# simone7monaco/NO-NODE-comparison

Measured on NVIDIA B200. Metric: train trajectories/s (EGNO 20-body, fwd+bwd+Adam), higher is better.
Workload: dtype f32

## Files before the change

### include/nbody_b200.h

```cpp
#ifndef NBODY_B200_H
#define NBODY_B200_H

#include <stdint.h>

#ifdef __cplusplus
extern "C" {
#endif

#define NB_HIDDEN 64
#define NB_MAX_EDGE_FEA 4
#define NB_MAX_T 16
#define NB_MAX_NODES 100

#define NB_OK 0
#define NB_ERR_INVALID (-1)
#define NB_ERR_CUDA (-2)

typedef struct NbEgnoConfig {
  int32_t B;
  int32_t N;
  int32_t T;
  int32_t n_layers;
  int32_t num_modes;
  int32_t in_node_nf;
// ... 64 lines not shown
                      const float* saved, const float* g_x_out, const float* g_h_out, const float* g_v_out,
                      float* grad_params, float* g_x_in, float* g_v_in, float* g_h_in, float* workspace, void* stream);

int64_t nb_segno_input_grad_workspace_floats(const NbSegnoConfig* cfg);
int nb_segno_backward_ex(const NbSegnoConfig* cfg, const float* params, const float* his, const float* edge_attr,
                         const float* saved, const float* g_x_out, const float* g_h_out, const float* g_v_out,
                         float* grad_params, float* g_x_in, float* g_v_in, float* g_h_in, float* g_his,
                         float* g_edge_attr, float* workspace, float* input_grad_workspace, void* stream);

int nb_segno_embed_forward(const NbSegnoConfig* cfg, const float* params, int64_t rows, const float* his, float* h,
                           void* stream);
int64_t nb_segno_embed_backward_workspace_floats(const NbSegnoConfig* cfg, int64_t rows);
int nb_segno_embed_backward(const NbSegnoConfig* cfg, int64_t rows, const float* his, const float* g_h, float* grad_params,
                            float* workspace, void* stream);
int nb_segno_merge_forward(int32_t mode, int64_t n, int32_t L, int32_t frame, const float* h_all, const float* x_all,
                           const float* v_all, const float* h_int, const float* x_int, const float* v_int,
                           const float* attn_params, float* h_out, float* x_out, float* v_out, float* alpha, void* stream);
int64_t nb_segno_merge_backward_workspace_floats(int64_t n);
int nb_segno_merge_backward(int32_t mode, int64_t n, int32_t L, int32_t frame, const float* h_all, const float* x_all,
                            const float* v_all, const float* h_int, const float* x_int, const float* v_int,
                            const float* attn_params, const float* alpha, const float* g_h, const float* g_x,
                            const float* g_v, float* g_h_all, float* g_x_all, float* g_v_all, float* g_h_int,
                            float* g_x_int, float* g_v_int, float* g_attn, int32_t accumulate, float* workspace,
                            void* stream);
int nb_accumulate(int64_t n, float* dst, const float* src, void* stream);

int nb_check_canonical_edges(const int64_t* row, const int64_t* col, int64_t n_edges, int32_t B, int32_t N,
                             int32_t* flag_dev, void* stream);


int nb_egcl_edge_forward(int32_t n_gt, int32_t B, int32_t N, int32_t n_edge_fea, int32_t clamp_per_edge,
                         const float* x, const float* P, const float* Q, const float* edge_fea, const float* w1,
                         int32_t ldw1, int32_t col_rad, int32_t col_ef, const float* W2, const float* b2,
                         const float* W3, const float* b3, const float* w4, const float* b4, float* M, float* Fsum,
                         void* stream);

int64_t nb_egcl_edge_backward_workspace_floats(int32_t n_gt, int32_t N);
int nb_egcl_edge_backward(int32_t n_gt, int32_t B, int32_t N, int32_t n_edge_fea, int32_t clamp_per_edge,
                          const float* x, const float* P, const float* Q, const float* edge_fea, const float* w1,
                          int32_t ldw1, int32_t col_rad, int32_t col_ef, const float* W2, const float* b2,
                          const float* W3, const float* b3, const float* w4, const float* b4, const float* gM,
                          const float* gFsum, float* gP, float* gQ, float* gx, float* gw, float* workspace,
                          void* stream);

long long nb_launch_count(void);
#define NB_PROFILE_CATEGORIES 8
int nb_profile_enable(int enable);
int nb_profile_read(double* ms , long long* counts );

int nb_set_edge_impl(int impl);
int nb_get_edge_impl(void);
int nb_set_edge_fwd3(int on);
int nb_get_edge_fwd3(void);
int nb_set_node_impl(int impl);
int nb_get_node_impl(void);
int nb_set_node_fused(int on);
int nb_get_node_fused(void);
int nb_set_segno_fused(int on);
int nb_get_segno_fused(void);

int nb_nbody_features(int32_t B, int32_t N, int32_t with_charge, const float* loc, const float* vel, const float* charges,
                      const float* edge_attr_o, float* nodes, float* loc_mean, float* edge_attr, void* stream);
int nb_nbody_energy(int32_t kind, int32_t F, int32_t B, int32_t N, float G, const float* loc, const float* vel,
                    const float* charges, float* energy, void* stream);

int64_t nb_traj_mse_workspace_floats(int32_t T);
int nb_traj_mse(int32_t T, int64_t rows, int32_t target_layout, int32_t only_first, const float* pred, const float* target,
                float* losses, float* loss, float* grad, float* workspace, void* stream);

int nb_sim_charged(int32_t B, int32_t N, int32_t T, int32_t sample_freq, double dt, double strength, double max_force,
                   double box_size, const double* loc0, const double* vel0, const double* charges, double* loc, double* vel,
                   void* stream);
int nb_sim_gravity(int32_t B, int32_t N, int32_t T, int32_t sample_freq, double dt, double G, double softening,
                   const double* pos0, const double* vel0, const double* mass, double* pos, double* vel, double* force,
                   void* stream);

int nb_adam_step(int64_t n, float* params, const float* grads, float* exp_avg, float* exp_avg_sq, float* step,
                 int32_t tick, double lr, double beta1, double beta2, double eps, double weight_decay, double grad_scale,
                 void* stream);
int nb_adam_step_peers(int64_t n, float* params, const void* const* peer_grads, int32_t npeer, float* exp_avg,
                       float* exp_avg_sq, float* step, int32_t tick, double lr, double beta1, double beta2, double eps,
                       double weight_decay, double grad_scale, void* stream);

int nb_tc_selftest(int32_t mode, const float* A, const float* W, float* out, void* stream);

int nb_silu_selftest(int64_t n, const float* x, float* out_mufu, float* out_fma, void* stream);

#ifdef __cplusplus
}
#endif
#endif
```

### no-node-comparison_b200/_cabi.py

```python
from __future__ import annotations

import ctypes as C

c_f = C.c_void_p


class NbEgnoConfig(C.Structure):
    _fields_ = [("B", C.c_int32), ("N", C.c_int32), ("T", C.c_int32), ("n_layers", C.c_int32),
                ("num_modes", C.c_int32), ("in_node_nf", C.c_int32), ("in_edge_nf", C.c_int32),
                ("time_emb_dim", C.c_int32), ("use_time_conv", C.c_int32), ("num_inputs", C.c_int32)]


class NbSegnoConfig(C.Structure):
    _fields_ = [("B", C.c_int32), ("N", C.c_int32), ("T", C.c_int32), ("in_node_nf", C.c_int32),
                ("in_edge_nf", C.c_int32), ("recurrent", C.c_int32), ("coords_weight", C.c_float),
                ("h_given", C.c_int32)]


EXPORTS = {
    "nb_version": (C.c_int, []),
    "nb_last_error": (C.c_char_p, []),
    "nb_egno_param_count": (C.c_int64, [C.POINTER(NbEgnoConfig)]),
    "nb_segno_param_count": (C.c_int64, [C.POINTER(NbSegnoConfig)]),
    "nb_egno_saved_floats": (C.c_int64, [C.POINTER(NbEgnoConfig)]),
    "nb_egno_workspace_floats": (C.c_int64, [C.POINTER(NbEgnoConfig), C.c_int]),
    "nb_segno_saved_floats": (C.c_int64, [C.POINTER(NbSegnoConfig)]),
    "nb_segno_workspace_floats": (C.c_int64, [C.POINTER(NbSegnoConfig), C.c_int]),
    "nb_egno_forward": (C.c_int, [C.POINTER(NbEgnoConfig)] + [c_f] * 14),
    "nb_egno_backward": (C.c_int, [C.POINTER(NbEgnoConfig)] + [c_f] * 15),
    "nb_segno_forward": (C.c_int, [C.POINTER(NbSegnoConfig)] + [c_f] * 11),
    "nb_segno_backward": (C.c_int, [C.POINTER(NbSegnoConfig)] + [c_f] * 13),
    "nb_egno_input_grad_workspace_floats": (C.c_int64, [C.POINTER(NbEgnoConfig)]),
    "nb_egno_backward_ex": (C.c_int, [C.POINTER(NbEgnoConfig)] + [c_f] * 19),
    "nb_egno_forward_ft": (C.c_int, [C.POINTER(NbEgnoConfig)] + [c_f] * 14),
    "nb_egno_backward_ft": (C.c_int, [C.POINTER(NbEgnoConfig)] + [c_f] * 21),
    "nb_segno_input_grad_workspace_floats": (C.c_int64, [C.POINTER(NbSegnoConfig)]),
    "nb_segno_backward_ex": (C.c_int, [C.POINTER(NbSegnoConfig)] + [c_f] * 16),
    "nb_segno_embed_forward": (C.c_int, [C.POINTER(NbSegnoConfig), c_f, C.c_int64, c_f, c_f, c_f]),
    "nb_segno_embed_backward_workspace_floats": (C.c_int64, [C.POINTER(NbSegnoConfig), C.c_int64]),
    "nb_segno_embed_backward": (C.c_int, [C.POINTER(NbSegnoConfig), C.c_int64] + [c_f] * 5),
    "nb_segno_merge_forward": (C.c_int, [C.c_int32, C.c_int64, C.c_int32, C.c_int32] + [c_f] * 12),
    "nb_segno_merge_backward_workspace_floats": (C.c_int64, [C.c_int64]),
    "nb_segno_merge_backward": (C.c_int, [C.c_int32, C.c_int64, C.c_int32, C.c_int32] + [c_f] * 18 + [C.c_int32, c_f, c_f]),
    "nb_accumulate": (C.c_int, [C.c_int64, c_f, c_f, c_f]),
    "nb_check_canonical_edges": (C.c_int, [c_f, c_f, C.c_int64, C.c_int32, C.c_int32, c_f, c_f]),
    "nb_egcl_edge_forward": (C.c_int, [C.c_int32] * 5 + [c_f] * 5 + [C.c_int32] * 3 + [c_f] * 9),
    "nb_egcl_edge_backward_workspace_floats": (C.c_int64, [C.c_int32, C.c_int32]),
    "nb_egcl_edge_backward": (C.c_int, [C.c_int32] * 5 + [c_f] * 5 + [C.c_int32] * 3 + [c_f] * 14),
    "nb_nbody_features": (C.c_int, [C.c_int32] * 3 + [c_f] * 8),
    "nb_nbody_energy": (C.c_int, [C.c_int32] * 4 + [C.c_float] + [c_f] * 5),
    "nb_sim_charged": (C.c_int, [C.c_int32] * 4 + [C.c_double] * 4 + [c_f] * 6),
    "nb_sim_gravity": (C.c_int, [C.c_int32] * 4 + [C.c_double] * 3 + [c_f] * 7),
    "nb_traj_mse_workspace_floats": (C.c_int64, [C.c_int32]),
    "nb_traj_mse": (C.c_int, [C.c_int32, C.c_int64, C.c_int32, C.c_int32] + [c_f] * 7),
    "nb_adam_step": (C.c_int, [C.c_int64] + [c_f] * 5 + [C.c_int32] + [C.c_double] * 6 + [c_f]),
    "nb_adam_step_peers": (C.c_int, [C.c_int64, c_f, C.POINTER(C.c_void_p), C.c_int32] + [c_f] * 3 + [C.c_int32] + [C.c_double] * 6 + [c_f]),
    "nb_launch_count": (C.c_longlong, []),
    "nb_profile_enable": (C.c_int, [C.c_int]),
    "nb_profile_read": (C.c_int, [C.POINTER(C.c_double), C.POINTER(C.c_longlong)]),
    "nb_set_edge_impl": (C.c_int, [C.c_int]),
    "nb_set_node_impl": (C.c_int, [C.c_int]),
    "nb_get_node_impl": (C.c_int, []),
    "nb_set_node_fused": (C.c_int, [C.c_int]),
    "nb_get_node_fused": (C.c_int, []),
    "nb_set_segno_fused": (C.c_int, [C.c_int]),
    "nb_get_segno_fused": (C.c_int, []),
    "nb_get_edge_impl": (C.c_int, []),
    "nb_set_edge_fwd3": (C.c_int, [C.c_int]),
    "nb_get_edge_fwd3": (C.c_int, []),
    "nb_tc_selftest": (C.c_int, [C.c_int32, c_f, c_f, c_f, c_f]),
    "nb_silu_selftest": (C.c_int, [C.c_int64, c_f, c_f, c_f, c_f]),
}


def declare(lib: C.CDLL) -> C.CDLL:
    for name, (res, args) in EXPORTS.items():
        fn = getattr(lib, name)
        fn.restype = res
        fn.argtypes = args
    return lib
```

### no-node-comparison_b200/csrc/nb_spectral.cuh

```cuda
#pragma once
#include "nb_common.cuh"

#define NB_MAX_MODES (NB_MAX_T / 2 + 1)
#define NB_MAX_COEF (2 * NB_MAX_MODES - 1)

struct NbTwiddle {
  int T, modes, ncoef;
  int nyq;
  float c[NB_MAX_MODES][NB_MAX_T];
  float s[NB_MAX_MODES][NB_MAX_T];
};

__host__ __device__ __forceinline__ int nb_coef_index(const NbTwiddle& tw, int m) { return m == 0 ? 0 : 2 * m - 1; }

struct NbDftArgs {
  NbTwiddle tw;
  int Nn0;
  const float* x;
  float* coef;
  const float* ycoef;
  float* out;
  const float* gout;
  float* gycoef;
  const float* gcoef;
// ... 323 lines not shown
      const int idx = tid + (half * 8 + it) * 256;
      w0[it] = __ldg(reinterpret_cast<const float2*>(W + (int64_t)idx * modes * 2));
      w1[it] = modes > 1 ? __ldg(reinterpret_cast<const float2*>(W + (int64_t)idx * modes * 2 + 2)) : make_float2(0.f, 0.f);
    }
#pragma unroll
    for (int it = 0; it < 8; ++it) {
      const int idx = tid + (half * 8 + it) * 256;
      const int i = idx >> 6, o = idx & 63;
      if (B0) {
        B0[idx] = w0[it].x;
        B1[idx] = w1[it].x;
        B2[idx] = w1[it].y;
      }
      if (T0) {
        T0[o * NB_TCV_LDT + i] = w0[it].x;
        T1[o * NB_TCV_LDT + i] = w1[it].x;
        T2[o * NB_TCV_LDT + i] = w1[it].y;
      }
    }
  }
}

__device__ __forceinline__ void nb_tconv_mix(const float* As, const float* B0, const float* B1, const float* B2, int ldb,
                                             int r, int c4, bool has1, bool pair1, float4& o0, float4& o1, float4& o2) {
  o0 = o1 = o2 = make_float4(0.f, 0.f, 0.f, 0.f);
  const float* a0 = As + r * NB_TCV_LDA;
  const float* a1 = a0 + NB_TCV_ROWS * NB_TCV_LDA;
  const float* a2 = a1 + NB_TCV_ROWS * NB_TCV_LDA;
#pragma unroll 2
  for (int k0 = 0; k0 < NB_H; k0 += 4) {
    const float4 v0 = nb_ld4(a0 + k0);
    const float4 v1 = has1 ? nb_ld4(a1 + k0) : make_float4(0.f, 0.f, 0.f, 0.f);
    const float4 v2 = pair1 ? nb_ld4(a2 + k0) : make_float4(0.f, 0.f, 0.f, 0.f);
    const float x0[4] = {v0.x, v0.y, v0.z, v0.w}, x1[4] = {v1.x, v1.y, v1.z, v1.w}, x2[4] = {v2.x, v2.y, v2.z, v2.w};
#pragma unroll
    for (int kk = 0; kk < 4; ++kk) {
      const int k = k0 + kk;
      o0 = nb_f4_fma(x0[kk], nb_ld4(B0 + k * ldb + c4 * 4), o0);
      if (has1) {
        const float4 b1 = nb_ld4(B1 + k * ldb + c4 * 4);
        o1 = nb_f4_fma(x1[kk], b1, o1);
        if (pair1) {
          const float4 b2 = nb_ld4(B2 + k * ldb + c4 * 4);
          o1 = nb_f4_fma(x2[kk], b2, o1);
          o2 = nb_f4_fma(x1[kk], b2, o2);
          o2 = nb_f4_fma(-x2[kk], b1, o2);
        }
      }
    }
  }
}

template <int MAXT>
__global__ void __launch_bounds__(256, 3) k_tconv_fwd(NbTconvArgs a) {
  NB_PDL_ENTER();
  NB_DYN_SMEM(sm);
  float* B0 = sm;
  float* B1 = B0 + NB_H * NB_H;
  float* B2 = B1 + NB_H * NB_H;
  float* As = B2 + NB_H * NB_H;
  const int tid = threadIdx.x, r = tid >> 4, c4 = tid & 15;
  const NbTwiddle& tw = a.tw;
  const bool has1 = tw.modes > 1, pair1 = has1 && tw.nyq != 1;
  const int64_t plane = (int64_t)a.Nn0 * NB_H;
  const float invT = 1.0f / (float)tw.T;
  const int ngroups = (a.Nn0 + NB_TCV_ROWS - 1) / NB_TCV_ROWS;
  float4 xs[MAXT];
  {
    const int row = blockIdx.x * NB_TCV_ROWS + r;
    const bool act = (int)blockIdx.x < ngroups && row < a.Nn0;
    const int64_t off = (int64_t)row * NB_H + c4 * 4;
#pragma unroll
    for (int t = 0; t < MAXT; ++t)
      if (t < tw.T) xs[t] = act ? nb_ld4(a.x + t * plane + off) : make_float4(0.f, 0.f, 0.f, 0.f);
  }
  nb_tconv_stage_w(B0, B1, B2, nullptr, nullptr, nullptr, a.W, tw.modes, tid);
  for (int grp = blockIdx.x; grp < ngroups; grp += gridDim.x) {
    const int row = grp * NB_TCV_ROWS + r;
    const bool act = row < a.Nn0;
    const int64_t off = (int64_t)row * NB_H + c4 * 4;
    if (grp != (int)blockIdx.x) {
#pragma unroll
      for (int t = 0; t < MAXT; ++t)
        if (t < tw.T) xs[t] = act ? nb_ld4(a.x + t * plane + off) : make_float4(0.f, 0.f, 0.f, 0.f);
    }
    float4 C0 = make_float4(0.f, 0.f, 0.f, 0.f), C1 = C0, S1 = C0;
#pragma unroll
    for (int t = 0; t < MAXT; ++t)
      if (t < tw.T) {
        C0 = nb_f4_fma(tw.c[0][t], xs[t], C0);
        if (has1) C1 = nb_f4_fma(tw.c[1][t], xs[t], C1);
        if (pair1) S1 = nb_f4_fma(tw.s[1][t], xs[t], S1);
      }
    __syncthreads();
    nb_st4(As + r * NB_TCV_LDA + c4 * 4, C0);
    nb_st4(As + (NB_TCV_ROWS + r) * NB_TCV_LDA + c4 * 4, C1);
    nb_st4(As + (2 * NB_TCV_ROWS + r) * NB_TCV_LDA + c4 * 4, S1);
    __syncthreads();
    float4 P0, P1, Q1;
    nb_tconv_mix(As, B0, B1, B2, NB_H, r, c4, has1, pair1, P0, P1, Q1);
    if (act) {
      const float s1 = pair1 ? 2.f * invT : invT;
      uint32_t m0 = 0u, m1 = 0u;
#pragma unroll
      for (int t = 0; t < MAXT; ++t)
        if (t < tw.T) {
          float4 y = make_float4(P0.x * invT, P0.y * invT, P0.z * invT, P0.w * invT);
          if (has1) y = nb_f4_fma(s1 * tw.c[1][t], P1, y);
          if (pair1) y = nb_f4_fma(-s1 * tw.s[1][t], Q1, y);
          nb_st4(a.out + t * plane + off, make_float4(xs[t].x + nb_leaky(y.x), xs[t].y + nb_leaky(y.y),
                                                      xs[t].z + nb_leaky(y.z), xs[t].w + nb_leaky(y.w)));
          const uint32_t bits = (y.x > 0.f ? 1u : 0u) | (y.y > 0.f ? 2u : 0u) | (y.z > 0.f ? 4u : 0u) | (y.w > 0.f ? 8u : 0u);
          if (t < 8) m0 |= bits << (4 * t);
          else m1 |= bits << (4 * (t - 8));
        }
      if (a.mask) {
        a.mask[((int64_t)row * 16 + c4) * 2] = m0;
        a.mask[((int64_t)row * 16 + c4) * 2 + 1] = m1;
      }
    }
  }
}

template <int MAXT>
__global__ void __launch_bounds__(256, 2) k_tconv_bwd(NbTconvArgs a) {
  NB_PDL_ENTER();
  NB_DYN_SMEM(sm);
  float* T0 = sm;
  float* T1 = T0 + NB_H * NB_TCV_LDT;
  float* T2 = T1 + NB_H * NB_TCV_LDT;
  float* As = T2 + NB_H * NB_TCV_LDT;
  const int tid = threadIdx.x, r = tid >> 4, c4 = tid & 15;
  const NbTwiddle& tw = a.tw;
  const bool has1 = tw.modes > 1, pair1 = has1 && tw.nyq != 1;
  const int64_t plane = (int64_t)a.Nn0 * NB_H;
  const float invT = 1.0f / (float)tw.T;
  const float s1 = pair1 ? 2.f * invT : invT;
  const int ngroups = (a.Nn0 + NB_TCV_ROWS - 1) / NB_TCV_ROWS;
  float4 gq[MAXT];
  {
    const int row = blockIdx.x * NB_TCV_ROWS + r;
    const bool act = (int)blockIdx.x < ngroups && row < a.Nn0;
    const int64_t off = (int64_t)row * NB_H + c4 * 4;
#pragma unroll
    for (int t = 0; t < MAXT; ++t)
      if (t < tw.T) gq[t] = act ? nb_ld4(a.gout + t * plane + off) : make_float4(0.f, 0.f, 0.f, 0.f);
  }
  nb_tconv_stage_w(nullptr, nullptr, nullptr, T0, T1, T2, a.W, tw.modes, tid);
  for (int grp = blockIdx.x; grp < ngroups; grp += gridDim.x) {
    const int row = grp * NB_TCV_ROWS + r;
    const bool act = row < a.Nn0;
    const int64_t off = (int64_t)row * NB_H + c4 * 4;
    if (grp != (int)blockIdx.x) {
#pragma unroll
      for (int t = 0; t < MAXT; ++t)
        if (t < tw.T) gq[t] = act ? nb_ld4(a.gout + t * plane + off) : make_float4(0.f, 0.f, 0.f, 0.f);
    }
    const uint32_t mk0 = act ? a.mask[((int64_t)row * 16 + c4) * 2] : 0u, mk1 = act ? a.mask[((int64_t)row * 16 + c4) * 2 + 1] : 0u;
    float4 C0 = make_float4(0.f, 0.f, 0.f, 0.f), C1 = C0, S1 = C0, gP0 = C0, gP1 = C0, gQ1 = C0;
#pragma unroll
    for (int t = 0; t < MAXT; ++t)
      if (t < tw.T) {
        const float4 xv = act ? nb_ld4(a.x + t * plane + off) : make_float4(0.f, 0.f, 0.f, 0.f);
        C0 = nb_f4_fma(tw.c[0][t], xv, C0);
        if (has1) C1 = nb_f4_fma(tw.c[1][t], xv, C1);
        if (pair1) S1 = nb_f4_fma(tw.s[1][t], xv, S1);
        const uint32_t bits = (t < 8 ? mk0 >> (4 * t) : mk1 >> (4 * (t - 8))) & 15u;
        const float4 g = gq[t];
        const float4 gy = make_float4(g.x * ((bits & 1u) ? 1.f : 0.01f), g.y * ((bits & 2u) ? 1.f : 0.01f),
                                      g.z * ((bits & 4u) ? 1.f : 0.01f), g.w * ((bits & 8u) ? 1.f : 0.01f));
        gP0 = nb_f4_fma(invT * tw.c[0][t], gy, gP0);
        if (has1) gP1 = nb_f4_fma(s1 * tw.c[1][t], gy, gP1);
        if (pair1) gQ1 = nb_f4_fma(-s1 * tw.s[1][t], gy, gQ1);
      }
    if (act) {
      nb_st4(a.coef + off, C0);
      if (has1) nb_st4(a.coef + plane + off, C1);
      if (pair1) nb_st4(a.coef + 2 * plane + off, S1);
      nb_st4(a.gycoef + off, gP0);
      if (has1) nb_st4(a.gycoef + plane + off, gP1);
      if (pair1) nb_st4(a.gycoef + 2 * plane + off, gQ1);
    }
    __syncthreads();
    nb_st4(As + r * NB_TCV_LDA + c4 * 4, gP0);
    nb_st4(As + (NB_TCV_ROWS + r) * NB_TCV_LDA + c4 * 4, gP1);
    nb_st4(As + (2 * NB_TCV_ROWS + r) * NB_TCV_LDA + c4 * 4, gQ1);
    __syncthreads();
    float4 gC0, gC1, gS1;
    nb_tconv_mix(As, T0, T1, T2, NB_TCV_LDT, r, c4, has1, pair1, gC0, gC1, gS1);
    if (act) {
#pragma unroll
      for (int t = 0; t < MAXT; ++t)
        if (t < tw.T) {
          float4 g = gq[t];
          g = nb_f4_fma(tw.c[0][t], gC0, g);
          if (has1) g = nb_f4_fma(tw.c[1][t], gC1, g);
          if (pair1) g = nb_f4_fma(tw.s[1][t], gS1, g);
          nb_st4(a.gx + t * plane + off, g);
        }
    }
  }
}
```

### no-node-comparison_b200/csrc/nbody_b200.cu

```cuda
#include <math.h>
#include <stdarg.h>
#include <stdio.h>
#include <string.h>

#include "nb_common.cuh"
#include "nb_node.cuh"
#include "nb_spectral.cuh"
#include "nb_rollout.cuh"
#include "nb_sim.cuh"
#include "nb_edge.cuh"
#include "nb_tc.cuh"
#include "nb_edge_tc.cuh"
#include "nb_edge_sel.cuh"
#include "nb_node_tc.cuh"
#include "nb_segno_fused.cuh"
#include "nb_merge.cuh"
#include "nb_egno_node.cuh"
#include <cstdlib>

#define NB_LAUNCH_COUNTED(...)                             \
  do {                                                     \
    __atomic_fetch_add(&g_launches, 1LL, __ATOMIC_RELAXED); \
    NB_LAUNCH(__VA_ARGS__);                                \
  } while (0)
// ... 948 lines not shown
}

static int egno_tc_mix(const EgnoCtx& X, int l, const float* coef, float* ycoef) {
  const int modes = X.c->num_modes;
  const float* W = X.params + X.lo.L[l].tc;
  const int64_t plane = X.Nn0 * NB_H;
  const int64_t sk = (int64_t)NB_H * modes * 2, sn = (int64_t)modes * 2;
  NbGemmArgs jobs[2 * NB_MAX_T];
  int nj = 0;
  for (int m = 0; m < modes; ++m) {
    int ci = nb_coef_index(X.tw, m);
    const float* Wr = W + m * 2;
    const float* Wi = W + m * 2 + 1;
    if (m == 0 || m == X.tw.nyq) {
      NbGemmArgs a = gemm_args((int)X.Nn0);
      a.nsrc = 1; a.src[0] = gsrc(coef + ci * plane, NB_H, 0, Wr, sk, sn);
      a.out = ycoef + ci * plane;
      jobs[nj++] = a;
    } else {
      NbGemmArgs a = gemm_args((int)X.Nn0);
      a.nsrc = 2;
      a.src[0] = gsrc(coef + ci * plane, NB_H, 0, Wr, sk, sn);
      a.src[1] = gsrc(coef + (ci + 1) * plane, NB_H, 0, Wi, sk, sn);
      a.out = ycoef + ci * plane;
      jobs[nj++] = a;
      NbGemmArgs b = gemm_args((int)X.Nn0);
      b.nsrc = 2;
      b.src[0] = gsrc(coef + ci * plane, NB_H, 0, Wi, sk, sn);
      b.src[1] = gsrc(coef + (ci + 1) * plane, NB_H, 0, Wr, sk, sn, -1.f);
      b.out = ycoef + (ci + 1) * plane;
      jobs[nj++] = b;
    }
  }
  return launch_gemm_batch(jobs, nj, X.st, true);
}

static NbDftArgs dft_args(const EgnoCtx& X) {
  NbDftArgs d;
  memset(&d, 0, sizeof(d));
  d.tw = X.tw;
  d.Nn0 = (int)X.Nn0;
  return d;
}

static inline bool egno_tconv_fused(const EgnoCtx& X) { return X.c->num_modes <= 2; }
static NbTconvArgs tconv_args(const EgnoCtx& X, int l) {
  NbTconvArgs t;
  memset(&t, 0, sizeof(t));
  t.tw = X.tw;
  t.Nn0 = (int)X.Nn0;
  t.W = X.params + X.lo.L[l].tc;
  return t;
}
static inline int tconv_grid(const EgnoCtx& X, int per_sm) {
  return imin(cdiv(X.Nn0, NB_TCV_ROWS), (int64_t)per_sm * nb_num_sms());
}

static bool egno_node_fused(const EgnoCtx& X) {
#ifndef NB_EMU
  static int off = -1;
  if (off < 0) { const char* e = getenv("NB_B200_EGNO_NODE_FUSED"); off = (e && e[0] == '0') ? 1 : 0; }
  return !off && g_node_fused && g_node_impl == 1 && g_wimg.n == EGNO_WIMG_PER_LAYER * X.c->n_layers;
#else
  (void)X;
  return false;
#endif
}

static int egno_pq(const EgnoCtx& X, int l, const float* h1, float* P, float* Q) {
  const EgnoLayerOff& L = X.lo.L[l];
  const int E = X.lo.E;
#ifndef NB_EMU
  if (egno_node_fused(X)) {
    NbEgnoPairArgs pa;
    memset(&pa, 0, sizeof(pa));
    pa.rows = (int)X.Nn; pa.img = g_wimg.img[EGNO_WIMG_PER_LAYER * l]; pa.A0 = h1; pa.bias = X.params + L.e_b1; pa.O0 = P; pa.O1 = Q;
    NB_SET_SMEM(k_egno_pair<true>, NB_EPR_SMEM);
    int pi = prof_begin(2, X.st);
    NB_LAUNCH_COUNTED(k_egno_pair<true>, (unsigned)imin(cdiv(X.Nn, NB_TILE), 2 * nb_num_sms()), NB_THREADS, NB_EPR_SMEM, X.st, pa);
    prof_end(2, pi, X.st);
    return nb_check_launch("k_egno_pair");
  }
#endif
  NbGemmArgs a = gemm_args((int)X.Nn);
  a.nsrc = 1; a.src[0] = gsrc(h1, NB_H, 0, X.params + L.e_w1 + 1, 1, E);
  a.bias = X.params + L.e_b1; a.out = P;
  NbGemmArgs b = gemm_args((int)X.Nn);
  b.nsrc = 1; b.src[0] = gsrc(h1, NB_H, 0, X.params + L.e_w1 + 1 + NB_H, 1, E);
  b.out = Q;
  NbGemmArgs ab[2] = {a, b};
  return launch_gemm_batch(ab, 2, X.st);
}

static NbEdgeW egno_edge_w(const EgnoCtx& X, int l) {
  const EgnoLayerOff& L = X.lo.L[l];
  NbEdgeW w;
  w.W1 = X.params + L.e_w1; w.ldw1 = X.lo.E; w.col_rad = 0; w.col_ef = 1 + 2 * NB_H;
  w.W2 = X.params + L.e_w2; w.b2 = X.params + L.e_b2; w.W3 = X.params + L.c_w1; w.b3 = X.params + L.c_b1;
  w.w4 = X.params + L.c_w2; w.b4 = X.params + L.c_b2;
  return w;
}

static int egno_forward(const NbEgnoConfig* cfg, const float* params, const float* x, const float* nodes,
                        const float* edge_fea, const float* v, const float* loc_mean, const EgnoTimes& times,
                        float* x_out, float* v_out, float* h_out, float* saved, float* workspace, void* stream) {
  NB_RANGE("nb_egno_forward");
  EgnoCtx X;
  NB_TRY(egno_ctx_init(&X, cfg, params, stream));
// ... 2 lines not shown
  const int64_t nh = align64(Nn * NB_H), cf = egno_coef_floats(cfg), lf = align64(egno_layer_floats(Nn, X.Nn0));
  WimgGuard wimg_guard;
  NB_TRY(egno_weight_images(X, workspace));
  float* ttab = workspace + wimg_floats(EGNO_WIMG_PER_LAYER * Ln);
  float* P = ttab + egno_table_floats(cfg);
  float* Q = P + nh;
  float* coef = Q + nh;
  float* ycoef = coef + cf;
  float* infer = ycoef + cf;
  auto bufs = [&](int l) { return egno_layer_bufs(saved ? saved + (int64_t)l * lf : infer + (int64_t)(l & 1) * lf, Nn); };

  EgnoLayerBufs b0 = bufs(0);
  {
    NbEmbedArgs e;
    NB_TRY(egno_embed_inputs(cfg, X.lo, e, nodes, times, ttab, P, Q, stream));
    {
      NbGemmArgs ga = gemm_args((int)Nn);
      ga.nsrc = 1; ga.src[0] = gsrc(P, NB_H, 0, params + X.lo.emb_w, 1, X.lo.F);
      ga.src[0].kmax = X.lo.F < NB_H ? X.lo.F : NB_H;
      if (X.lo.F > NB_H) {
        ga.nsrc = 2; ga.src[1] = gsrc(Q, NB_H, 0, params + X.lo.emb_w + NB_H, 1, X.lo.F);
        ga.src[1].kmax = X.lo.F - NB_H;
      }
      ga.bias = params + X.lo.emb_b; ga.out = b0.h0;
      NB_TRY(launch_gemm(ga, stream));
    }
    const NbFrameMap fm = egno_frame_map(cfg);
    NB_LAUNCH_COUNTED(k_replicate3, (unsigned)ew_grid(Nn * 3), 256, 0, stream, x, b0.x0, (int)(Nn0 * 3), T, fm);
    NB_LAUNCH_COUNTED(k_replicate3, (unsigned)ew_grid(Nn * 3), 256, 0, stream, v, b0.v0, (int)(Nn0 * 3), T, fm);
    NB_TRY(nb_check_launch("k_replicate3"));
  }

  const float* v_prev = b0.v0;
  for (int l = 0; l < Ln; ++l) {
    EgnoLayerBufs b = bufs(l);
    const EgnoLayerOff& L = X.lo.L[l];
    const float* v0 = v_prev;
    float *h1 = b.h1, *x1 = b.x1, *v1 = b.v1;
    void* side = stream;
    if (cfg->use_time_conv) {
      {
        NbTcxArgs t;
        memset(&t, 0, sizeof(t));
        t.tw = X.tw; t.n3 = (int)(Nn0 * 3); t.x0 = b.x0; t.v0 = v0; t.mean = loc_mean; t.W = params + L.tcx;
        { const NbFrameMap fmx = egno_frame_map(cfg); for (int tt = 0; tt < NB_MAX_T; ++tt) t.tmap[tt] = fmx.m[tt]; }
        t.x1 = x1; t.v1 = v1;
        side = side_fork(stream);
        NB_LAUNCH_COUNTED(k_tcx_fwd, (unsigned)ew_grid(Nn0 * 3), 256, 0, side, t);
        NB_TRY(nb_check_launch("k_tcx_fwd"));
      }
      if (egno_tconv_fused(X)) {
        NbTconvArgs tc = tconv_args(X, l);
        tc.x = b.h0; tc.out = h1; tc.mask = saved ? b.tmask : nullptr;
        int pi = prof_begin(4, stream);
        if (T <= 10) {
          NB_SET_SMEM(k_tconv_fwd<10>, NB_TCONV_FWD_SMEM);
          NB_LAUNCH_COUNTED(k_tconv_fwd<10>, (unsigned)tconv_grid(X, 3), 256, NB_TCONV_FWD_SMEM, stream, tc);
        } else {
          NB_SET_SMEM(k_tconv_fwd<NB_MAX_T>, NB_TCONV_FWD_SMEM);
          NB_LAUNCH_COUNTED(k_tconv_fwd<NB_MAX_T>, (unsigned)tconv_grid(X, 3), 256, NB_TCONV_FWD_SMEM, stream, tc);
        }
        prof_end(4, pi, stream);
        NB_TRY(nb_check_launch("k_tconv_fwd"));
      } else {
        NbDftArgs d = dft_args(X);
        d.x = b.h0; d.coef = coef;
        NB_LAUNCH_COUNTED(k_dft_fwd, (unsigned)ew_grid(Nn0 * 16), 256, 0, stream, d);
        NB_TRY(nb_check_launch("k_dft_fwd"));
        NB_TRY(egno_tc_mix(X, l, coef, ycoef));
        d.ycoef = ycoef; d.out = h1;
        NB_LAUNCH_COUNTED(k_idft_fwd, (unsigned)ew_grid(Nn0 * 16), 256, 0, stream, d);
        NB_TRY(nb_check_launch("k_idft_fwd"));
      }
    } else {
      h1 = b.h0; x1 = b.x0;
      cudaMemcpyAsync(v1, v0, Nn * 3 * sizeof(float), cudaMemcpyDeviceToDevice, (cudaStream_t)stream);
    }
    float* Pl = saved ? b.P : P;
    float* Ql = saved ? b.Q : Q;
    NB_TRY(egno_pq(X, l, h1, Pl, Ql));
    side_join(side, stream);
    NbEdgeFwdArgs ea;
    ea.g = edge_geom(T * cfg->B, cfg->B, cfg->N, cfg->in_edge_nf, 0);
    egno_geom_frames(cfg, ea.g);
    ea.w = egno_edge_w(X, l);
    ea.x = x1; ea.P = Pl; ea.Q = Ql; ea.ef = edge_fea; ea.M = b.M; ea.Fsum = b.Fsum;
    NB_TRY(launch_edge_fwd(ea, stream));
    float* h_next = (l + 1 < Ln) ? bufs(l + 1).h0 : h_out;
    float* x_next = (l + 1 < Ln) ? bufs(l + 1).x0 : x_out;
    bool node_fused = false;
#ifndef NB_EMU
    node_fused = egno_node_fused(X);
    if (node_fused) {
      NbEgnoNodeFwdArgs na;
      memset(&na, 0, sizeof(na));
      na.rows = (int)Nn; na.N = cfg->N; na.img = g_wimg.img[EGNO_WIMG_PER_LAYER * l + 2];
      na.h = h1; na.M = b.M; na.b5 = params + L.n_b1; na.b6 = params + L.n_b2; na.bv1 = params + L.v_b1;
      na.wv2 = params + L.v_w2; na.bv2 = params + L.v_b2; na.x = x1; na.v = v1; na.Fsum = b.Fsum;
      na.U5 = saved ? b.U5 : nullptr; na.UV = saved ? b.UV : nullptr;
      na.h_out = h_next; na.x_out = x_next;
      NB_SET_SMEM(k_egno_node_fwd, NB_ENF_SMEM);
      int pi = prof_begin(6, stream);
      NB_LAUNCH_COUNTED(k_egno_node_fwd, (unsigned)imin(cdiv(Nn, NB_TILE), 2 * nb_num_sms()), NB_THREADS, NB_ENF_SMEM, stream, na);
      prof_end(6, pi, stream);
      NB_TRY(nb_check_launch("k_egno_node_fwd"));
    }
#endif
    if (!node_fused) {
      NbGemmArgs a = gemm_args((int)Nn);
      a.nsrc = 2;
      a.src[0] = gsrc(h1, NB_H, 0, params + L.n_w1, 1, 2 * NB_H);
      a.src[1] = gsrc(b.M, NB_H, 0, params + L.n_w1 + NB_H, 1, 2 * NB_H);
      a.bias = params + L.n_b1; a.out_pre = b.U5;
      NbGemmArgs u = gemm_args((int)Nn);
      u.nsrc = 1; u.src[0] = gsrc(h1, NB_H, 0, params + L.v_w1, 1, NB_H);
      u.bias = params + L.v_b1; u.out_pre = b.UV;
// ... 280 lines not shown
        prof_end(2, pi, stream);
        NB_TRY(nb_check_launch("k_egno_pair"));
      } else
#endif
      {
      NbGemmArgs a = gemm_args((int)Nn);
      a.nsrc = 2;
      a.src[0] = gsrc(gP, NB_H, 0, params + L.e_w1 + 1, X.lo.E, 1);
      a.src[1] = gsrc(gQ, NB_H, 0, params + L.e_w1 + 1 + NB_H, X.lo.E, 1);
      a.out = ghA; a.accumulate = 1;
      NB_TRY(launch_gemm(a, stream));
      }
      NB_TRY(wgrad_to((int)Nn, 1, wpair(gP, h1), wpair(nullptr, nullptr), grad_params, L.e_w1 + 1, X.lo.E, 1,
                      L.e_b1, 0, stream));
      NB_TRY(wgrad_to((int)Nn, 1, wpair(gQ, h1), wpair(nullptr, nullptr), grad_params, L.e_w1 + 1 + NB_H,
                      X.lo.E, 1, -1, 0, stream));
    }
    if (cfg->use_time_conv) {
      float* gx0 = gxb[gxi ^ 1];
      void* side = stream;
      if (egno_tconv_fused(X)) {
        NB_TRY(defer_flush(D, stream));
        side = side_fork(stream);
      }
      {
        NbTcxArgs t;
        memset(&t, 0, sizeof(t));
        t.tw = X.tw; t.n3 = (int)(Nn0 * 3); t.x0 = b.x0; t.v0 = v0; t.mean = loc_mean; t.W = params + L.tcx;
      { const NbFrameMap fmx = egno_frame_map(cfg); for (int tt = 0; tt < NB_MAX_T; ++tt) t.tmap[tt] = fmx.m[tt]; }
        t.gx1 = gx; t.gv1 = gvB; t.gx0 = gx0; t.gv0 = gvA;
        int grid = imin(cdiv(Nn0 * 3, 256), 2 * nb_num_sms());
        float* partial = q_alloc((int64_t)grid * 2 * 2 * modes * 2, stream);
        if (!partial) { nb_set_error("partial-sum workspace too small"); return NB_ERR_INVALID; }
        t.partial = partial;
        NB_LAUNCH_COUNTED(k_tcx_bwd, (unsigned)grid, 256, 0, side, t);
        NB_TRY(nb_check_launch("k_tcx_bwd"));
        if (g_loc_mean) {
          NB_LAUNCH_COUNTED(k_loc_mean_grad, (unsigned)ew_grid(Nn0 * 3), 256, 0, side, (const float*)gx, (const float*)gx0,
                            g_loc_mean, (int)(Nn0 * 3), T, l == Ln - 1 ? 0 : 1);
          NB_TRY(nb_check_launch("k_loc_mean_grad"));
        }
        NbFinArgs f;
        memset(&f, 0, sizeof(f));
        int nw = 2 * 2 * modes * 2;
        f.partial = partial; f.nparts = grid; f.plen = nw; f.dst = grad_params; f.nseg = 1;
        f.seg[0] = fseg(0, nw, nw, L.tcx, 0, 1);
        NB_TRY(launch_finalize(f, stream));
      }
      gxi ^= 1;
      gv_in = gvA;
      if (egno_tconv_fused(X)) {
        NbTconvArgs tc = tconv_args(X, l);
        tc.x = b.h0; tc.gout = ghA; tc.gx = ghB; tc.coef = coef; tc.gycoef = gycoef; tc.mask = b.tmask;
        int pi = prof_begin(4, stream);
        if (T <= 10) {
          NB_SET_SMEM(k_tconv_bwd<10>, NB_TCONV_BWD_SMEM);
          NB_LAUNCH_COUNTED(k_tconv_bwd<10>, (unsigned)tconv_grid(X, 2), 256, NB_TCONV_BWD_SMEM, stream, tc);
        } else {
          NB_SET_SMEM(k_tconv_bwd<NB_MAX_T>, NB_TCONV_BWD_SMEM);
          NB_LAUNCH_COUNTED(k_tconv_bwd<NB_MAX_T>, (unsigned)tconv_grid(X, 2), 256, NB_TCONV_BWD_SMEM, stream, tc);
        }
        prof_end(4, pi, stream);
        NB_TRY(nb_check_launch("k_tconv_bwd"));
        side_join(side, stream);
        const int64_t plane = Nn0 * NB_H;
        const int64_t tk = (int64_t)modes * 2, tn = (int64_t)NB_H * modes * 2;
        for (int m = 0; m < modes; ++m) {
          int ci = nb_coef_index(X.tw, m);
          const float *C = coef + ci * plane, *S = coef + (ci + 1) * plane;
          const float *gPm = gycoef + ci * plane, *gQm = gycoef + (ci + 1) * plane;
          const int64_t wr_off = L.tc + m * 2, wi_off = L.tc + m * 2 + 1;
          if (m == 0 || m == X.tw.nyq) {
            NB_TRY(wgrad_to((int)Nn0, 1, wpair(C, gPm), wpair(nullptr, nullptr), grad_params, wr_off, tn, tk, -1, 0, stream));
          } else {
            NB_TRY(wgrad_to((int)Nn0, 2, wpair(C, gPm), wpair(S, gQm, 0, -1.f), grad_params, wr_off, tn, tk, -1, 0, stream));
            NB_TRY(wgrad_to((int)Nn0, 2, wpair(S, gPm), wpair(C, gQm), grad_params, wi_off, tn, tk, -1, 0, stream));
          }
        }
      } else
      {
        NbDftArgs d = dft_args(X);
        d.x = b.h0; d.coef = coef;
        NB_LAUNCH_COUNTED(k_dft_fwd, (unsigned)ew_grid(Nn0 * 16), 256, 0, stream, d);
        NB_TRY(nb_check_launch("k_dft_fwd"));
        NB_TRY(egno_tc_mix(X, l, coef, ycoef));
        d.ycoef = ycoef; d.gout = ghA; d.gycoef = gycoef;
        NB_LAUNCH_COUNTED(k_idft_bwd, (unsigned)ew_grid(Nn0 * 16), 256, 0, stream, d);
        NB_TRY(nb_check_launch("k_idft_bwd"));
        const float* W = params + L.tc;
        const int64_t plane = Nn0 * NB_H;
        const int64_t tk = (int64_t)modes * 2, tn = (int64_t)NB_H * modes * 2;
        NbGemmArgs gj[2 * NB_MAX_T];
        int ngj = 0;
        for (int m = 0; m < modes; ++m) {
          int ci = nb_coef_index(X.tw, m);
          const float *Wr = W + m * 2, *Wi = W + m * 2 + 1;
          const float *C = coef + ci * plane, *S = coef + (ci + 1) * plane;
          const float *gPm = gycoef + ci * plane, *gQm = gycoef + (ci + 1) * plane;
          const int64_t wr_off = L.tc + m * 2, wi_off = L.tc + m * 2 + 1;
          if (m == 0 || m == X.tw.nyq) {
            NbGemmArgs a = gemm_args((int)Nn0);
            a.nsrc = 1; a.src[0] = gsrc(gPm, NB_H, 0, Wr, tk, tn);
            a.out = gcoef + ci * plane;
            gj[ngj++] = a;
            NB_TRY(wgrad_to((int)Nn0, 1, wpair(C, gPm), wpair(nullptr, nullptr), grad_params, wr_off, tn, tk,
                            -1, 0, stream));
          } else {
            NbGemmArgs a = gemm_args((int)Nn0);
            a.nsrc = 2;
            a.src[0] = gsrc(gPm, NB_H, 0, Wr, tk, tn);
            a.src[1] = gsrc(gQm, NB_H, 0, Wi, tk, tn);
            a.out = gcoef + ci * plane;
            gj[ngj++] = a;
            NbGemmArgs s2 = gemm_args((int)Nn0);
            s2.nsrc = 2;
            s2.src[0] = gsrc(gPm, NB_H, 0, Wi, tk, tn);
// ... 873 lines not shown
```

Baseline: 82350.

## Add streaming persistent temporal-conv kernels with register prefetch of next chunk

Adds new forward and backward temporal-convolution kernels that run one persistent block per SM. Each block walks its range of node rows in 32-row chunks and prefetches the next chunk's activations into registers while the current chunk's mode mixing runs from shared memory. The weights are staged into shared memory once per block rather than once per tile, which cuts redundant weight loads. In exchange, occupancy drops to one block per SM and register pressure rises from holding two chunks; the backward path is used only for T <= 10. The new path is on by default and can be switched off at runtime.

```diff
diff --git a/include/nbody_b200.h b/include/nbody_b200.h
--- a/include/nbody_b200.h
+++ b/include/nbody_b200.h
@@ -140,6 +140,8 @@
 int nb_get_edge_impl(void);
 int nb_set_edge_fwd3(int on);
 int nb_get_edge_fwd3(void);
+int nb_set_tconv_fast(int on);
+int nb_get_tconv_fast(void);
 int nb_set_node_impl(int impl);
 int nb_get_node_impl(void);
 int nb_set_node_fused(int on);
diff --git a/no-node-comparison_b200/_cabi.py b/no-node-comparison_b200/_cabi.py
--- a/no-node-comparison_b200/_cabi.py
+++ b/no-node-comparison_b200/_cabi.py
@@ -68,6 +68,8 @@
     "nb_get_edge_impl": (C.c_int, []),
     "nb_set_edge_fwd3": (C.c_int, [C.c_int]),
     "nb_get_edge_fwd3": (C.c_int, []),
+    "nb_set_tconv_fast": (C.c_int, [C.c_int]),
+    "nb_get_tconv_fast": (C.c_int, []),
     "nb_tc_selftest": (C.c_int, [C.c_int32, c_f, c_f, c_f, c_f]),
     "nb_silu_selftest": (C.c_int, [C.c_int64, c_f, c_f, c_f, c_f]),
 }
diff --git a/no-node-comparison_b200/csrc/nb_spectral.cuh b/no-node-comparison_b200/csrc/nb_spectral.cuh
--- a/no-node-comparison_b200/csrc/nb_spectral.cuh
+++ b/no-node-comparison_b200/csrc/nb_spectral.cuh
@@ -399,8 +399,7 @@
 }
 
 template <int MAXT>
-__global__ void __launch_bounds__(256, 3) k_tconv_fwd(NbTconvArgs a) {
-  NB_PDL_ENTER();
+__device__ __forceinline__ void nb_tconv_fwd_ref(const NbTconvArgs& a) {
   NB_DYN_SMEM(sm);
   float* B0 = sm;
   float* B1 = B0 + NB_H * NB_H;
@@ -470,8 +469,7 @@
 }
 
 template <int MAXT>
-__global__ void __launch_bounds__(256, 2) k_tconv_bwd(NbTconvArgs a) {
-  NB_PDL_ENTER();
+__device__ __forceinline__ void nb_tconv_bwd_ref(const NbTconvArgs& a) {
   NB_DYN_SMEM(sm);
   float* T0 = sm;
   float* T1 = T0 + NB_H * NB_TCV_LDT;
@@ -548,3 +546,246 @@
     }
   }
 }
+
+#define NB_TCV_SROWS 32
+#define NB_TCONV_FWD_SMEM_S ((3 * NB_H * NB_H + 3 * NB_TCV_SROWS * NB_TCV_LDA) * sizeof(float))
+#define NB_TCONV_BWD_SMEM_S ((3 * NB_H * NB_TCV_LDT + 3 * NB_TCV_SROWS * NB_TCV_LDA) * sizeof(float))
+struct NbTconvSpan {
+  int lo, hi, cs, nch;
+  __device__ __forceinline__ NbTconvSpan(int Nn0) {
+    lo = (int)((int64_t)blockIdx.x * Nn0 / gridDim.x);
+    hi = (int)((int64_t)(blockIdx.x + 1) * Nn0 / gridDim.x);
+    nch = (hi - lo + NB_TCV_SROWS - 1) / NB_TCV_SROWS;
+    cs = nch ? (hi - lo + nch - 1) / nch : 0;
+  }
+  __device__ __forceinline__ int row(int c, int r) const { return lo + c * cs + r; }
+  __device__ __forceinline__ bool active(int c, int r) const { return r < cs && row(c, r) < hi; }
+};
+
+template <int MAXT>
+__device__ __forceinline__ void nb_tconv_load(float4 (&v)[MAXT], const float* src, int T, int64_t plane, int64_t off, bool act) {
+#pragma unroll
+  for (int t = 0; t < MAXT; ++t)
+    if (t < T) v[t] = act ? nb_ld4(src + t * plane + off) : make_float4(0.f, 0.f, 0.f, 0.f);
+}
+
+__device__ __forceinline__ void nb_tconv_mix2(const float* As, const float* B0, const float* B1, const float* B2, int ldb,
+                                              int r0, int c4, bool has1, bool pair1, float4 (&o0)[2], float4 (&o1)[2],
+                                              float4 (&o2)[2]) {
+  const float* a0[2] = {As + r0 * NB_TCV_LDA, As + (r0 + 1) * NB_TCV_LDA};
+#pragma unroll
+  for (int j = 0; j < 2; ++j) o0[j] = o1[j] = o2[j] = make_float4(0.f, 0.f, 0.f, 0.f);
+#pragma unroll 2
+  for (int k0 = 0; k0 < NB_H; k0 += 4) {
+    float x0[2][4], x1[2][4], x2[2][4];
+#pragma unroll
+    for (int j = 0; j < 2; ++j) {
+      const float4 v0 = nb_ld4(a0[j] + k0);
+      const float4 v1 = has1 ? nb_ld4(a0[j] + NB_TCV_SROWS * NB_TCV_LDA + k0) : make_float4(0.f, 0.f, 0.f, 0.f);
+      const float4 v2 = pair1 ? nb_ld4(a0[j] + 2 * NB_TCV_SROWS * NB_TCV_LDA + k0) : make_float4(0.f, 0.f, 0.f, 0.f);
+      x0[j][0] = v0.x; x0[j][1] = v0.y; x0[j][2] = v0.z; x0[j][3] = v0.w;
+      x1[j][0] = v1.x; x1[j][1] = v1.y; x1[j][2] = v1.z; x1[j][3] = v1.w;
+      x2[j][0] = v2.x; x2[j][1] = v2.y; x2[j][2] = v2.z; x2[j][3] = v2.w;
+    }
+#pragma unroll
+    for (int kk = 0; kk < 4; ++kk) {
+      const int k = k0 + kk;
+      const float4 b0 = nb_ld4(B0 + k * ldb + c4 * 4);
+#pragma unroll
+      for (int j = 0; j < 2; ++j) o0[j] = nb_f4_fma(x0[j][kk], b0, o0[j]);
+      if (has1) {
+        const float4 b1 = nb_ld4(B1 + k * ldb + c4 * 4);
+        const float4 b2 = pair1 ? nb_ld4(B2 + k * ldb + c4 * 4) : make_float4(0.f, 0.f, 0.f, 0.f);
+#pragma unroll
+        for (int j = 0; j < 2; ++j) {
+          o1[j] = nb_f4_fma(x1[j][kk], b1, o1[j]);
+          if (pair1) {
+            o1[j] = nb_f4_fma(x2[j][kk], b2, o1[j]);
+            o2[j] = nb_f4_fma(x1[j][kk], b2, o2[j]);
+            o2[j] = nb_f4_fma(-x2[j][kk], b1, o2[j]);
+          }
+        }
+      }
+    }
+  }
+}
+
+template <int MAXT>
+__device__ __forceinline__ void nb_tconv_fwd_stream(const NbTconvArgs& a) {
+  NB_DYN_SMEM(sm);
+  float* B0 = sm;
+  float* B1 = B0 + NB_H * NB_H;
+  float* B2 = B1 + NB_H * NB_H;
+  float* As = B2 + NB_H * NB_H;
+  const int tid = threadIdx.x, r0 = (tid >> 4) * 2, c4 = tid & 15, wr = (tid >> 5) * 4;
+  const NbTwiddle& tw = a.tw;
+  const bool has1 = tw.modes > 1, pair1 = has1 && tw.nyq != 1;
+  const int64_t plane = (int64_t)a.Nn0 * NB_H;
+  const float invT = 1.0f / (float)tw.T;
+  const NbTconvSpan sp(a.Nn0);
+  float4 xs[2][MAXT], xn[2][MAXT];
+#pragma unroll
+  for (int j = 0; j < 2; ++j)
+    nb_tconv_load<MAXT>(xs[j], a.x, tw.T, plane, (int64_t)sp.row(0, r0 + j) * NB_H + c4 * 4, sp.active(0, r0 + j));
+  nb_tconv_stage_w(B0, B1, B2, nullptr, nullptr, nullptr, a.W, tw.modes, tid);
+  for (int c = 0; c < sp.nch; ++c) {
+    float4 C0[2], C1[2], S1[2];
+#pragma unroll
+    for (int j = 0; j < 2; ++j) {
+      C0[j] = C1[j] = S1[j] = make_float4(0.f, 0.f, 0.f, 0.f);
+#pragma unroll
+      for (int t = 0; t < MAXT; ++t)
+        if (t < tw.T) {
+          C0[j] = nb_f4_fma(tw.c[0][t], xs[j][t], C0[j]);
+          if (has1) C1[j] = nb_f4_fma(tw.c[1][t], xs[j][t], C1[j]);
+          if (pair1) S1[j] = nb_f4_fma(tw.s[1][t], xs[j][t], S1[j]);
+        }
+    }
+    __syncthreads();
+#pragma unroll
+    for (int j = 0; j < 2; ++j) {
+      nb_st4(As + (r0 + j) * NB_TCV_LDA + c4 * 4, C0[j]);
+      nb_st4(As + (NB_TCV_SROWS + r0 + j) * NB_TCV_LDA + c4 * 4, C1[j]);
+      nb_st4(As + (2 * NB_TCV_SROWS + r0 + j) * NB_TCV_LDA + c4 * 4, S1[j]);
+    }
+    if (c + 1 < sp.nch) {
+#pragma unroll
+      for (int j = 0; j < 2; ++j)
+        nb_tconv_load<MAXT>(xn[j], a.x, tw.T, plane, (int64_t)sp.row(c + 1, r0 + j) * NB_H + c4 * 4, sp.active(c + 1, r0 + j));
+    }
+    __syncthreads();
+    float4 P0[2], P1[2], Q1[2];
+    if (sp.active(c, wr)) nb_tconv_mix2(As, B0, B1, B2, NB_H, r0, c4, has1, pair1, P0, P1, Q1);
+    const float s1 = pair1 ? 2.f * invT : invT;
+#pragma unroll
+    for (int j = 0; j < 2; ++j) {
+      const int row = sp.row(c, r0 + j);
+      if (!sp.active(c, r0 + j)) continue;
+      const int64_t off = (int64_t)row * NB_H + c4 * 4;
+      uint32_t m0 = 0u, m1 = 0u;
+#pragma unroll
+      for (int t = 0; t < MAXT; ++t)
+        if (t < tw.T) {
+          float4 y = make_float4(P0[j].x * invT, P0[j].y * invT, P0[j].z * invT, P0[j].w * invT);
+          if (has1) y = nb_f4_fma(s1 * tw.c[1][t], P1[j], y);
+          if (pair1) y = nb_f4_fma(-s1 * tw.s[1][t], Q1[j], y);
+          const float4 xv = nb_ld4(a.x + t * plane + off);
+          nb_st4(a.out + t * plane + off, make_float4(xv.x + nb_leaky(y.x), xv.y + nb_leaky(y.y),
+                                                      xv.z + nb_leaky(y.z), xv.w + nb_leaky(y.w)));
+          const uint32_t bits = (y.x > 0.f ? 1u : 0u) | (y.y > 0.f ? 2u : 0u) | (y.z > 0.f ? 4u : 0u) | (y.w > 0.f ? 8u : 0u);
+          if (t < 8) m0 |= bits << (4 * t);
+          else m1 |= bits << (4 * (t - 8));
+        }
+      if (a.mask) {
+        a.mask[((int64_t)row * 16 + c4) * 2] = m0;
+        a.mask[((int64_t)row * 16 + c4) * 2 + 1] = m1;
+      }
+    }
+#pragma unroll
+    for (int j = 0; j < 2; ++j)
+#pragma unroll
+      for (int t = 0; t < MAXT; ++t) xs[j][t] = xn[j][t];
+  }
+}
+
+template <int MAXT>
+__device__ __forceinline__ void nb_tconv_bwd_stream(const NbTconvArgs& a) {
+  NB_DYN_SMEM(sm);
+  float* T0 = sm;
+  float* T1 = T0 + NB_H * NB_TCV_LDT;
+  float* T2 = T1 + NB_H * NB_TCV_LDT;
+  float* As = T2 + NB_H * NB_TCV_LDT;
+  const int tid = threadIdx.x, r0 = (tid >> 4) * 2, c4 = tid & 15, wr = (tid >> 5) * 4;
+  const NbTwiddle& tw = a.tw;
+  const bool has1 = tw.modes > 1, pair1 = has1 && tw.nyq != 1;
+  const int64_t plane = (int64_t)a.Nn0 * NB_H;
+  const float invT = 1.0f / (float)tw.T;
+  const float s1 = pair1 ? 2.f * invT : invT;
+  const NbTconvSpan sp(a.Nn0);
+  static_assert(MAXT <= 10, "the streaming backward holds two chunks of two rows: T <= 10");
+  float4 xs[2][MAXT], gq[2][MAXT];
+  uint32_t mk[2][2];
+  auto load = [&](int c, int j) {
+    const bool act = sp.active(c, r0 + j);
+    const int row = sp.row(c, r0 + j);
+    const int64_t off = (int64_t)row * NB_H + c4 * 4;
+    nb_tconv_load<MAXT>(gq[j], a.gout, tw.T, plane, off, act);
+    nb_tconv_load<MAXT>(xs[j], a.x, tw.T, plane, off, act);
+    mk[j][0] = act ? a.mask[((int64_t)row * 16 + c4) * 2] : 0u;
+    mk[j][1] = act ? a.mask[((int64_t)row * 16 + c4) * 2 + 1] : 0u;
+  };
+  load(0, 0);
+  load(0, 1);
+  nb_tconv_stage_w(nullptr, nullptr, nullptr, T0, T1, T2, a.W, tw.modes, tid);
+  for (int c = 0; c < sp.nch; ++c) {
+    float4 gP0[2], gP1[2], gQ1[2];
+#pragma unroll
+    for (int j = 0; j < 2; ++j) {
+      const int64_t off = (int64_t)sp.row(c, r0 + j) * NB_H + c4 * 4;
+      float4 C0 = make_float4(0.f, 0.f, 0.f, 0.f), C1 = C0, S1 = C0;
+      gP0[j] = gP1[j] = gQ1[j] = C0;
+#pragma unroll
+      for (int t = 0; t < MAXT; ++t)
+        if (t < tw.T) {
+          const float4 xv = xs[j][t];
+          C0 = nb_f4_fma(tw.c[0][t], xv, C0);
+          if (has1) C1 = nb_f4_fma(tw.c[1][t], xv, C1);
+          if (pair1) S1 = nb_f4_fma(tw.s[1][t], xv, S1);
+          const uint32_t bits = (t < 8 ? mk[j][0] >> (4 * t) : mk[j][1] >> (4 * (t - 8))) & 15u;
+          const float4 g = gq[j][t];
+          const float4 gy = make_float4(g.x * ((bits & 1u) ? 1.f : 0.01f), g.y * ((bits & 2u) ? 1.f : 0.01f),
+                                        g.z * ((bits & 4u) ? 1.f : 0.01f), g.w * ((bits & 8u) ? 1.f : 0.01f));
+          gP0[j] = nb_f4_fma(invT * tw.c[0][t], gy, gP0[j]);
+          if (has1) gP1[j] = nb_f4_fma(s1 * tw.c[1][t], gy, gP1[j]);
+          if (pair1) gQ1[j] = nb_f4_fma(-s1 * tw.s[1][t], gy, gQ1[j]);
+        }
+      if (sp.active(c, r0 + j)) {
+        nb_st4(a.coef + off, C0);
+        if (has1) nb_st4(a.coef + plane + off, C1);
+        if (pair1) nb_st4(a.coef + 2 * plane + off, S1);
+        nb_st4(a.gycoef + off, gP0[j]);
+        if (has1) nb_st4(a.gycoef + plane + off, gP1[j]);
+        if (pair1) nb_st4(a.gycoef + 2 * plane + off, gQ1[j]);
+      }
+    }
+    __syncthreads();
+#pragma unroll
+    for (int j = 0; j < 2; ++j) {
+      nb_st4(As + (r0 + j) * NB_TCV_LDA + c4 * 4, gP0[j]);
+      nb_st4(As + (NB_TCV_SROWS + r0 + j) * NB_TCV_LDA + c4 * 4, gP1[j]);
+      nb_st4(As + (2 * NB_TCV_SROWS + r0 + j) * NB_TCV_LDA + c4 * 4, gQ1[j]);
+    }
+    if (c + 1 < sp.nch) { load(c + 1, 0); load(c + 1, 1); }
+    __syncthreads();
+    float4 gC0[2], gC1[2], gS1[2];
+    if (sp.active(c, wr)) nb_tconv_mix2(As, T0, T1, T2, NB_TCV_LDT, r0, c4, has1, pair1, gC0, gC1, gS1);
+#pragma unroll
+    for (int j = 0; j < 2; ++j) {
+      if (!sp.active(c, r0 + j)) continue;
+      const int64_t off = (int64_t)sp.row(c, r0 + j) * NB_H + c4 * 4;
+#pragma unroll
+      for (int t = 0; t < MAXT; ++t)
+        if (t < tw.T) {
+          float4 g = nb_ld4(a.gout + t * plane + off);
+          g = nb_f4_fma(tw.c[0][t], gC0[j], g);
+          if (has1) g = nb_f4_fma(tw.c[1][t], gC1[j], g);
+          if (pair1) g = nb_f4_fma(tw.s[1][t], gS1[j], g);
+          nb_st4(a.gx + t * plane + off, g);
+        }
+    }
+  }
+}
+
+template <int MAXT, bool STREAM>
+__global__ void __launch_bounds__(256, STREAM ? 1 : 3) k_tconv_fwd(NbTconvArgs a) {
+  NB_PDL_ENTER();
+  if constexpr (STREAM) nb_tconv_fwd_stream<MAXT>(a);
+  else nb_tconv_fwd_ref<MAXT>(a);
+}
+
+template <int MAXT, bool STREAM>
+__global__ void __launch_bounds__(256, STREAM ? 1 : 2) k_tconv_bwd(NbTconvArgs a) {
+  NB_PDL_ENTER();
+  if constexpr (STREAM) nb_tconv_bwd_stream<MAXT>(a);
+  else nb_tconv_bwd_ref<MAXT>(a);
+}
diff --git a/no-node-comparison_b200/csrc/nbody_b200.cu b/no-node-comparison_b200/csrc/nbody_b200.cu
--- a/no-node-comparison_b200/csrc/nbody_b200.cu
+++ b/no-node-comparison_b200/csrc/nbody_b200.cu
@@ -1024,8 +1024,27 @@
   t.W = X.params + X.lo.L[l].tc;
   return t;
 }
-static inline int tconv_grid(const EgnoCtx& X, int per_sm) {
-  return imin(cdiv(X.Nn0, NB_TCV_ROWS), (int64_t)per_sm * nb_num_sms());
+static int g_tconv_fast = 1;
+extern "C" int nb_set_tconv_fast(int on) { g_tconv_fast = on ? 1 : 0; return NB_OK; }
+extern "C" int nb_get_tconv_fast(void) { return g_tconv_fast; }
+
+static int launch_tconv(const EgnoCtx& X, const NbTconvArgs& tc, bool bwd, void* stream) {
+  typedef void (*TconvKernel)(NbTconvArgs);
+  const bool t10 = X.c->T <= 10;
+  bool fast = g_tconv_fast != 0;
+  TconvKernel k;
+  if (bwd) fast = fast && t10;
+  if (bwd) k = fast ? k_tconv_bwd<10, true> : (t10 ? k_tconv_bwd<10, false> : k_tconv_bwd<NB_MAX_T, false>);
+  else k = fast ? (t10 ? k_tconv_fwd<10, true> : k_tconv_fwd<NB_MAX_T, true>)
+                : (t10 ? k_tconv_fwd<10, false> : k_tconv_fwd<NB_MAX_T, false>);
+  const size_t smem = fast ? (bwd ? NB_TCONV_BWD_SMEM_S : NB_TCONV_FWD_SMEM_S) : (bwd ? NB_TCONV_BWD_SMEM : NB_TCONV_FWD_SMEM);
+  const int grid = fast ? (int)imin(cdiv(X.Nn0, NB_TCV_ROWS), (int64_t)nb_num_sms())
+                        : (int)imin(cdiv(X.Nn0, NB_TCV_ROWS), (int64_t)(bwd ? 2 : 3) * nb_num_sms());
+  NB_SET_SMEM(k, smem);
+  int pi = prof_begin(4, stream);
+  NB_LAUNCH_COUNTED(k, (unsigned)grid, 256, smem, stream, tc);
+  prof_end(4, pi, stream);
+  return nb_check_launch(bwd ? "k_tconv_bwd" : "k_tconv_fwd");
 }
 
 static bool egno_node_fused(const EgnoCtx& X) {
@@ -1134,16 +1153,7 @@
       if (egno_tconv_fused(X)) {
         NbTconvArgs tc = tconv_args(X, l);
         tc.x = b.h0; tc.out = h1; tc.mask = saved ? b.tmask : nullptr;
-        int pi = prof_begin(4, stream);
-        if (T <= 10) {
-          NB_SET_SMEM(k_tconv_fwd<10>, NB_TCONV_FWD_SMEM);
-          NB_LAUNCH_COUNTED(k_tconv_fwd<10>, (unsigned)tconv_grid(X, 3), 256, NB_TCONV_FWD_SMEM, stream, tc);
-        } else {
-          NB_SET_SMEM(k_tconv_fwd<NB_MAX_T>, NB_TCONV_FWD_SMEM);
-          NB_LAUNCH_COUNTED(k_tconv_fwd<NB_MAX_T>, (unsigned)tconv_grid(X, 3), 256, NB_TCONV_FWD_SMEM, stream, tc);
-        }
-        prof_end(4, pi, stream);
-        NB_TRY(nb_check_launch("k_tconv_fwd"));
+        NB_TRY(launch_tconv(X, tc, false, stream));
       } else {
         NbDftArgs d = dft_args(X);
         d.x = b.h0; d.coef = coef;
@@ -1530,16 +1540,7 @@
       if (egno_tconv_fused(X)) {
         NbTconvArgs tc = tconv_args(X, l);
         tc.x = b.h0; tc.gout = ghA; tc.gx = ghB; tc.coef = coef; tc.gycoef = gycoef; tc.mask = b.tmask;
-        int pi = prof_begin(4, stream);
-        if (T <= 10) {
-          NB_SET_SMEM(k_tconv_bwd<10>, NB_TCONV_BWD_SMEM);
-          NB_LAUNCH_COUNTED(k_tconv_bwd<10>, (unsigned)tconv_grid(X, 2), 256, NB_TCONV_BWD_SMEM, stream, tc);
-        } else {
-          NB_SET_SMEM(k_tconv_bwd<NB_MAX_T>, NB_TCONV_BWD_SMEM);
-          NB_LAUNCH_COUNTED(k_tconv_bwd<NB_MAX_T>, (unsigned)tconv_grid(X, 2), 256, NB_TCONV_BWD_SMEM, stream, tc);
-        }
-        prof_end(4, pi, stream);
-        NB_TRY(nb_check_launch("k_tconv_bwd"));
+        NB_TRY(launch_tconv(X, tc, true, stream));
         side_join(side, stream);
         const int64_t plane = Nn0 * NB_H;
         const int64_t tk = (int64_t)modes * 2, tn = (int64_t)NB_H * modes * 2;
```

Result: slower. 78650 (median of 6 runs) (-4.5%).
